# zyddnys/sd_animation_optical_flow

Measured on AMD Instinct MI355X. Metric: frame-pairs/sec (flow+warp+mask) at 512x768, higher is better.
Workload: dtype f32

## Files before the change

### include/ofx.h

```cpp
#ifndef OFX_H
#define OFX_H

#include <stddef.h>
#include <stdint.h>

#ifdef __cplusplus
extern "C" {
#endif

#define OFX_VERSION 100

#define OFX_EINVAL   (-1)
#define OFX_EALIGN   (-2)
#define OFX_ENOMEM   (-3)
#define OFX_EKEY     (-4)
#define OFX_ENODEV   (-5)

int ofx_version(void);
const char* ofx_error_string(int code);

int ofx_prof_enable(int on);
int ofx_prof_collect(char* json_out, size_t cap);

#define OFX_WARP_BILINEAR  0
// ... 109 lines not shown
#define OFX_EPI_FLOW    3

#define OFX_PREC_FP32   0
#define OFX_PREC_BF16X3 1
#define OFX_PREC_BF16X3_W 2
#define OFX_PREC_BF16X6_W 4
#define OFX_PREC_BF16X6 3
#define OFX_PREC_F16 5

typedef struct ofx_conv_desc {
    const float* in0; int ld0; int c0;
    const float* in1; int ld1; int c1;
    const float* w;
    const float* scale;
    const float* shift;
    float* out; int ldo;
    const float* res; int ldres;
    const float* nmean; const float* nrstd;
    const float* addend; int ldadd;
    float* aux_z; float* aux_rh; float* aux_h; int ldh;
    float* aux_coords; float* aux_flow4;
    long a_zs, w_zs, o_zs; int nz;
    int B, Hin, Win, Hout, Wout, Cout, KH, KW, stride, padH, padW;
    int act, epi;
    int tile;
    int precision;
    void* splitk_ws;
    size_t splitk_ws_bytes;
    const float* wino_w;
    const float* wino4_w;
} ofx_conv_desc;
#define OFX_CONV_TILE_WINOGRAD 1
#define OFX_CONV_TILE_WINOGRAD4 2

int ofx_conv2d(const ofx_conv_desc* d, void* stream);
typedef struct ofx_conv_plan {
    int path;
    int bm, bn, wm, wn, bk;
    int prec;
    int ks;
    int ksplit;
    int mode;
    int mtiles, ntiles, group_m;
    int stats_rows;
} ofx_conv_plan;
int ofx_conv2d_plan(const ofx_conv_desc* d, size_t stats_cap_floats, int want_pool, ofx_conv_plan* out);
long ofx_pack_conv_weight(const float* w_oihw, int Cout, int Cin, int KH, int KW, int cin_pad,
                          float* out);
int ofx_split_conv_weight(const float* packed, long n_floats, float* out);
long ofx_wino_conv_weight(const float* w_oihw, int Cout, int Cin, float* out);
long ofx_wino15_conv_weight(const float* w_oihw, int Cout, int Cin, int KH, int KW, float* out);
long ofx_wino44_conv_weight(const float* w_oihw, int Cout, int Cin, float* out);
int ofx_split_conv_weight3(const float* packed, long n_floats, float* out);

int ofx_inorm_stats(const float* x, int ld, float* mean, float* rstd, float* scratch,
                    int B, long HW, int C, float eps, void* stream);
int ofx_conv2d_stats(const ofx_conv_desc* d, float* part, size_t part_floats, int* rows_per_image, void* stream);
int ofx_inorm_finalize(const float* part, float* mean, float* rstd, int B, int rows, long HW, int C, float eps, void* stream);
int ofx_inorm_apply(const float* x, const float* mean, const float* rstd, const float* res,
                    const float* res_mean, const float* res_rstd, float* out, int B, long HW, int C,
                    int relu, void* stream);
int ofx_preprocess_u8(const uint8_t* img, float* out, long npix, int bgr, void* stream);

int ofx_corr_slice_floats(int h_l, int w_l);
int ofx_corr_volume(const float* f1, const float* f2, float* const* pyr, int B, int h, int w, int D,
                    int levels, void* stream);
// ... 75 lines not shown
```

### sd_animation_optical_flow_amd/csrc/conv.hip

```cpp
#include "ofx_internal.h"

#include <algorithm>
#include <cstdlib>
#include <cstring>
#include <type_traits>

namespace {

struct ConvK {
    const float* in0;
    const float* in1;
    const float* w;
    const float* scale;
    const float* shift;
    const float* addend;
    float* out;
    const float* res;
    const float* nmean;
    const float* nrstd;
    float* aux_z;
    float* aux_rh;
    float* aux_h;
    float* aux_coords;
    float* aux_flow4;
// ... 1090 lines not shown
        if (k.patch) return launch_tile_uk<BM, BN, WM, WN, BK, PREC, KS, SK, 2>(k, epi, norm, nz, s, ev);
    }
    if constexpr (tile_has_scalar(BN, PREC)) {
        if (k.uk) return launch_tile_uk<BM, BN, WM, WN, BK, PREC, KS, SK, 1>(k, epi, norm, nz, s, ev);
    }
    return launch_tile_uk<BM, BN, WM, WN, BK, PREC, KS, SK, 0>(k, epi, norm, nz, s, ev);
}

struct TileInst {
    int bm, bn, wm, wn, bk, prec, ks;
    bool sk;
    int (*launch)(const ConvK&, int epi, bool norm, int nz, hipStream_t, hipEvent_t);
};
#define OFX_TILE(BM, BN, WM, WN, BK, PREC, KS, SK) {BM, BN, WM, WN, BK, PREC, KS, SK, &launch_tile<BM, BN, WM, WN, BK, PREC, KS, SK>}
const TileInst kTiles[] = {
#ifndef OFX_CONV_LEAN
    OFX_TILE(128, 128, 64, 64, 16, 3, 1, false), OFX_TILE(128, 128, 64, 64, 16, 2, 1, false), OFX_TILE(128, 128, 64, 64, 16, 1, 1, false),
    OFX_TILE(128, 128, 64, 64, 16, 4, 1, false), OFX_TILE(128, 64, 64, 32, 16, 4, 1, false),  OFX_TILE(64, 64, 32, 32, 16, 4, 1, false),
    OFX_TILE(128, 64, 64, 32, 16, 3, 1, false),  OFX_TILE(64, 64, 32, 32, 16, 3, 1, false),   OFX_TILE(128, 128, 64, 64, 32, 1, 1, false),
    OFX_TILE(128, 64, 64, 32, 16, 2, 1, false),  OFX_TILE(128, 64, 64, 32, 16, 1, 1, false),  OFX_TILE(64, 64, 32, 32, 16, 2, 1, false),
    OFX_TILE(64, 64, 32, 32, 16, 1, 1, false),
    OFX_TILE(128, 128, 64, 64, 16, 5, 1, false), OFX_TILE(128, 64, 64, 32, 16, 5, 1, false),  OFX_TILE(64, 64, 32, 32, 16, 5, 1, false),
    OFX_TILE(128, 128, 64, 64, 32, 5, 1, false), OFX_TILE(128, 64, 64, 32, 32, 5, 1, false),  OFX_TILE(64, 64, 32, 32, 32, 5, 1, false),
#endif
    OFX_TILE(128, 128, 64, 64, 16, 0, 1, false), OFX_TILE(256, 64, 64, 64, 16, 0, 1, false),  OFX_TILE(128, 192, 64, 96, 16, 0, 1, false),
    OFX_TILE(128, 96, 32, 96, 16, 0, 1, false),  OFX_TILE(128, 64, 64, 32, 16, 0, 1, false),  OFX_TILE(128, 128, 64, 64, 32, 0, 1, false),
    OFX_TILE(128, 64, 64, 32, 32, 0, 1, false),  OFX_TILE(128, 32, 32, 32, 32, 0, 1, false),  OFX_TILE(64, 64, 32, 32, 16, 0, 1, false),
    OFX_TILE(64, 64, 32, 32, 32, 0, 1, true),    OFX_TILE(64, 64, 32, 32, 32, 0, 2, false),   OFX_TILE(64, 64, 32, 32, 32, 0, 1, false),
};
#undef OFX_TILE

struct ConvKnobs {
    bool no_wino = false, no_wino15 = false;
    bool no_wino44 = false;
    bool old_small = false;
    bool no_splitk = false;
    long sk_max_tiles = 2048;
    bool no_uk = false, no_patch = false;
    double patch_max_waste = 1.09;
    long vol_group_m = 0;
    long pair_max = 320;
    long f16_bk = 0;
};

const ConvKnobs& conv_knobs() {
    static const ConvKnobs knobs = [] {
        auto flag = [](const char* name) { return getenv(name) != nullptr; };
        auto number = [](const char* name, double lo, double hi, double dflt) {
            const char* e = getenv(name);
            char* end = nullptr;
            const double v = e ? strtod(e, &end) : 0.0;
            return e && end != e && !*end && v >= lo && v <= hi ? v : dflt;
        };
        ConvKnobs k;
        k.no_wino = flag("OFX_CONV_NO_WINOGRAD");
        k.no_wino15 = k.no_wino || flag("OFX_CONV_NO_WINOGRAD15");
        k.no_wino44 = k.no_wino || flag("OFX_CONV_NO_WINOGRAD4");
        k.old_small = flag("OFX_CONV_OLD_SMALL_TILES");
        k.no_splitk = flag("OFX_NO_SPLITK");
        k.no_uk = flag("OFX_CONV_NO_UK");
        k.no_patch = flag("OFX_CONV_NO_PATCH");
        auto count = [&](const char* name, long dflt) { const double v = number(name, 0, 0x7FFFFFFF, dflt); return v == (long)v ? (long)v : dflt; };
        k.sk_max_tiles = count("OFX_SK_MAX_TILES", k.sk_max_tiles);
        k.patch_max_waste = number("OFX_PATCH_MAX_WASTE", 1.0, 1e30, k.patch_max_waste);
        k.vol_group_m = count("OFX_VOL_GROUP_M", k.vol_group_m);
        k.pair_max = count("OFX_CONV_PAIR_MAX", k.pair_max);
        k.f16_bk = count("OFX_CONV_F16_BK", 0);
        if (k.f16_bk != 16 && k.f16_bk != 32) k.f16_bk = 0;
        return k;
    }();
    return knobs;
}

struct ConvPlan : ofx_conv_plan {
    int inst = -1;
    const char* name = nullptr;
    double flops = 0.0;
};

int conv_plan(const ofx_conv_desc* d, const ConvExtra& x, const ConvKnobs& kn, ConvPlan* p) {
    *p = ConvPlan{};
    p->ks = p->ksplit = p->group_m = 1;
    const int nz = d->nz > 1 ? d->nz : 1, cin = d->c0 + d->c1;
    const int K = d->KH * d->KW * cin, Kpad = ((K + kKAlign - 1) / kKAlign) * kKAlign;
    const long M = (long)d->B * d->Hout * d->Wout;
    const bool want_stats = x.stats_rows != nullptr, pool = x.pool.out != nullptr, fp32 = d->precision == OFX_PREC_FP32, f16 = d->precision == OFX_PREC_F16;
    p->name = nz > 1 ? "igemm_corr_volume"
              : d->epi == OFX_EPI_GRU_ZR ? "igemm_conv_gru_zr"
              : d->epi == OFX_EPI_GRU_Q  ? "igemm_conv_gru_q"
              : d->epi == OFX_EPI_FLOW   ? "igemm_conv_flow"
                                         : "igemm_conv";

    OfxWinoChoice wino;
    if (int st = ofx_conv_wino_choose(d, want_stats, x.stats_cap, pool, kn.no_wino, kn.no_wino15, kn.no_wino44, &wino)) return st;
    if (wino.path != kPathIgemm) {
        p->path = wino.path;
        p->stats_rows = wino.stats_rows;
        p->flops = wino.flops;
        return 0;
    }
    const bool one_d = (d->KH == 1 && d->KW == 5) || (d->KH == 5 && d->KW == 1);
    p->flops = 2.0 * (double)M * d->Cout * K * nz;

    int bm, bn;
    if (d->tile) {
        bm = (d->tile % 1000000) / 1000;
        bn = d->tile % 1000;
    } else {
        auto waste = [&](int t) { return (double)(((d->Cout + t - 1) / t) * t) / d->Cout; };
        if (d->Cout <= 32) bn = 32;
        else if (waste(128) <= 1.13 && !(waste(192) <= 1.0 && waste(128) > 1.05 && fp32 && !d->nmean && d->epi == OFX_EPI_PLAIN)) bn = 128;
        else if (waste(192) <= 1.05 && fp32 && !d->nmean && d->epi != OFX_EPI_FLOW) bn = 192;
        else if (waste(96) <= 1.05 && fp32 && d->epi == OFX_EPI_PLAIN) bn = 96;
        else if (waste(64) <= 1.13) bn = 64;
        else if (waste(32) < waste(64) - 0.1) bn = 32;
        else bn = 64;
        bm = 128;
        const long mt128 = (M + 127) / 128;
        auto blocks_of = [&](int t) { return mt128 * ((d->Cout + t - 1) / t) * nz; };
        constexpr long kFill = 768;
        const long blocks128 = blocks_of(bn);
        if (kn.old_small) {
            if (bn == 96 && blocks128 < 1024) bn = 32;
            if (bn >= 64 && blocks128 < 1024) bm = 64;
            if (bm == 64 && bn >= 128) bn = 64;
        } else if (bn >= 64 && blocks128 < kFill) {
            if (bn == 192 && d->epi == OFX_EPI_PLAIN && blocks_of(96) >= kFill) bn = 96;
            else if (bn >= 128 && blocks_of(64) >= kFill) bn = 64;
            else if (bn == 96) bn = 32;
// ... 183 lines not shown

int ofx_conv2d_ex(const ofx_conv_desc* d, const ConvExtra* extra, hipStream_t s) {
    const ConvExtra x = extra ? *extra : ConvExtra{};
    if (x.stats_rows) *x.stats_rows = 0;
    if (x.stop_taken) *x.stop_taken = false;
    long split_rows = 0;
    int st = conv_validate(d, x, &split_rows);
    if (st) return st;
    if (split_rows) {
        const long Mtot = (long)d->B * d->Hout * d->Wout;
        for (long r0 = 0; r0 < Mtot && !st; r0 += split_rows) {
            ofx_conv_desc part = *d;
            const long n = std::min(split_rows, Mtot - r0);
            part.B = 1; part.Hin = part.Hout = 1; part.Win = part.Wout = (int)n;
            part.in0 = d->in0 + r0 * d->ld0;
            if (d->in1) part.in1 = d->in1 + r0 * d->ld1;
            part.out = d->out + r0 * d->ldo;
            if (d->res) part.res = d->res + r0 * d->ldres;
            if (d->addend) part.addend = d->addend + r0 * d->ldadd;
            ConvExtra px;
            px.alpha = x.alpha;
            px.pool = x.pool;
            if (x.pool.out) px.pool.out = x.pool.out + r0 * x.pool.slice1;
            if (r0 + split_rows >= Mtot) { px.stop_event = x.stop_event; px.stop_taken = x.stop_taken; }
            st = ofx_conv2d_ex(&part, &px, s);
        }
        return st;
    }
    ConvPlan p;
    if ((st = conv_plan(d, x, conv_knobs(), &p))) return st;
    OfxProfScope prof(p.name, s);
    prof.flops(p.flops);
    if (p.path != kPathIgemm) {
        st = ofx_conv_wino_launch(d, p.path, x.alpha, p.stats_rows ? x.stats_part : nullptr, s, x.stop_event);
    } else {
        const bool pool = x.pool.out != nullptr;
        st = kTiles[p.inst].launch(conv_args(d, x, p), pool ? kEpiVolPool : d->epi, !pool && d->nmean != nullptr, d->nz > 1 ? d->nz : 1, s, x.stop_event);
    }
    if (st) return st;
    if (x.stats_rows) *x.stats_rows = p.stats_rows;
    if (x.stop_taken) *x.stop_taken = x.stop_event != nullptr;
    return 0;
}

extern "C" int ofx_conv2d(const ofx_conv_desc* d, void* stream) { return ofx_conv2d_ex(d, nullptr, (hipStream_t)stream); }

int ofx_conv2d_stats(const ofx_conv_desc* d, float* part, size_t part_floats, int* rows_per_image, void* stream) {
    OFX_REQUIRE(rows_per_image != nullptr, OFX_EINVAL);
    ConvExtra x;
    x.stats_part = part; x.stats_cap = part_floats; x.stats_rows = rows_per_image;
    return ofx_conv2d_ex(d, &x, (hipStream_t)stream);
}

extern "C" int ofx_conv2d_plan(const ofx_conv_desc* d, size_t stats_cap_floats, int want_pool, ofx_conv_plan* out) {
    OFX_REQUIRE(out != nullptr, OFX_EINVAL);
    int rows = 0;
    ConvExtra x;
    if (stats_cap_floats) { x.stats_cap = stats_cap_floats; x.stats_rows = &rows; }
    if (want_pool) { x.pool.out = reinterpret_cast<float*>(uintptr_t(16)); x.pool.wb0 = x.pool.wb1 = x.pool.slice1 = 1; }
    long split_rows = 0;
    int st = conv_validate(d, x, &split_rows);
    if (!st && split_rows) st = OFX_EINVAL;
    ConvPlan p;
    if (!st) st = conv_plan(d, x, conv_knobs(), &p);
    if (st) return st;
    *out = p;
    return 0;
// ... 65 lines not shown
```

### sd_animation_optical_flow_amd/csrc/conv_wino.hip

```cpp
#include "ofx_internal.h"

#include <cmath>
#include <cstdlib>
#include <cstring>

namespace {

constexpr int kWBK = 16;
constexpr int kLDV = kWBK + 4;
constexpr int kOOB = 0x7FFFFFF0;

template <int W_, int H_, int Y0, int X0> struct HaloGeom {
    static constexpr int W = W_, H = H_, y_org = Y0, x_org = X0;
    static constexpr int pix = W * H;
    static constexpr int items = pix * (kWBK / 4);
    static constexpr int slots = (items + 255) / 256;
};
template <bool VERT> struct Halo15 : HaloGeom<VERT ? 16 : 20, VERT ? 12 : 8, VERT ? -2 : 0, VERT ? 0 : -2> {
    static constexpr int ldh = VERT ? 16 : 20;
    static constexpr int floats = Halo15::pix * ldh;
    __device__ static int at(int pix) { return pix * ldh; }
};
struct Halo3x3 : HaloGeom<18, 10, -1, -1> {
    static constexpr int lpair = 36, lrow = 336;
// ... 483 lines not shown
            const float s12 = m1 + m2, d12 = m1 - m2, s34 = m3 + m4, d34 = m3 - m4, s56 = m5 + m6, d56 = m5 - m6;
            y[u][0] = m0 + s12 + s34 + s56;
            y[u][1] = d12 + 2.0f * d34 + 0.5f * d56;
            y[u][2] = s12 + 4.0f * s34 + 0.25f * s56;
            y[u][3] = d12 + 8.0f * d34 + 0.125f * d56 + m7;
        }
#pragma unroll
        for (int u = 0; u < 4; ++u)
#pragma unroll
            for (int i = 0; i < 4; ++i) {
                ad[u][i] = p.addend ? p.addend[pix[u][i] * p.ldadd + n] : 0.0f;
                x1[u][i] = EPI == OFX_EPI_GRU_ZR ? (r_half ? p.aux_h[pix[u][i] * p.ldh + n - hd] : 1.0f)
                           : EPI == OFX_EPI_GRU_Q ? p.aux_z[pix[u][i] * p.Cout + n] : 0.0f;
                x2[u][i] = EPI == OFX_EPI_GRU_Q ? p.aux_h[pix[u][i] * p.ldh + n] : 0.0f;
            }
#pragma unroll
        for (int u = 0; u < 4; ++u)
#pragma unroll
            for (int i = 0; i < 4; ++i) {
                const float v = y[u][i] * sc + sh + ad[u][i];
                if (EPI == OFX_EPI_PLAIN) {
                    p.out[pix[u][i] * p.ldo + n] = fmaxf(v, act_lo);
                } else if (EPI == OFX_EPI_GRU_ZR) {
                    const float g = ofx_sigmoid(v) * x1[u][i];
                    if (r_half) p.aux_rh[pix[u][i] * hd + n - hd] = g;
                    else p.aux_z[pix[u][i] * hd + n] = g;
                } else {
                    p.aux_h[pix[u][i] * p.ldh + n] = (1.0f - x1[u][i]) * x2[u][i] + x1[u][i] * ofx_tanh(v);
                }
            }
    }
}

struct Halo44 {
    static constexpr int W = 34, H = 18;
    static constexpr int lquad = 34, lrow = 308;
    static constexpr int floats = H * lrow;
    static constexpr int items = W * H * 2;
    static constexpr int threads = 768;
    static constexpr int slots = (items + threads - 1) / threads;
    __device__ __host__ static constexpr int at(int y, int x) { return y * lrow + (x >> 2) * lquad + (x & 3) * 8; }
    static constexpr int ltrow = 336;
    static constexpr int tfloats = 6 * 4 * ltrow;
    static constexpr int titems = 4 * W * 4;
};
constexpr int kLDX4 = 40;
constexpr int kXF4 = 12 * 4 * 16 * kLDX4;
constexpr int kStage44 = 2 * (Halo44::floats + Halo44::tfloats);
constexpr int kSmem44 = (kStage44 > kXF4 ? kStage44 : kXF4) * 4;
constexpr int kNorm44 = kSmem44 / 4 - kStage44;
constexpr int kNorm44MaxCin = kNorm44 / 2 / kWBK * kWBK;
constexpr int kSX4 = 2 * 24 * 32 * 2;
static_assert(kNorm44 >= 0 && kSX4 <= kXF4, "the fused options live in the plain kernel's LDS");

__global__ __launch_bounds__(768, 1) void wino44_conv_kernel(const WinoK p) {
    extern __shared__ __attribute__((aligned(16))) float smem44[];
    constexpr bool NORM = false, RES = false, STATS = false;
#include "conv_wino44_body.inl"
}

template <bool NORM, bool RES, bool STATS>
__global__ __launch_bounds__(768, 1) void wino44_fused_kernel(const WinoK p) {
    extern __shared__ __attribute__((aligned(16))) float smem44[];
#include "conv_wino44_body.inl"
}


using WinoKernel = void (*)(WinoK);

const WinoKernel kKernels22[8] = {wino_conv_kernel<false, false, false>, wino_conv_kernel<false, false, true>,
                                  wino_conv_kernel<false, true, false>,  nullptr,
                                  wino_conv_kernel<true, false, false>,  wino_conv_kernel<true, false, true>,
                                  wino_conv_kernel<true, true, false>,   nullptr};
const WinoKernel kKernels15[8] = {wino15_conv_kernel<true, OFX_EPI_PLAIN>,  wino15_conv_kernel<true, OFX_EPI_GRU_ZR>,
                                  wino15_conv_kernel<true, OFX_EPI_GRU_Q>,  wino15_conv_kernel<false, OFX_EPI_PLAIN>,
                                  wino15_conv_kernel<false, OFX_EPI_GRU_ZR>, wino15_conv_kernel<false, OFX_EPI_GRU_Q>,
                                  nullptr,                                  nullptr};
const WinoKernel kKernels44[8] = {wino44_conv_kernel,                       wino44_fused_kernel<false, false, true>,
                                  wino44_fused_kernel<false, true, false>,  nullptr,
                                  wino44_fused_kernel<true, false, false>,  wino44_fused_kernel<true, false, true>,
                                  wino44_fused_kernel<true, true, false>,   nullptr};

struct WinoAlg {
    bool one_d;
    int ph, pw;
    int points, outputs;
    int cblk;
    int threads, dyn_lds;
    const float* ofx_conv_desc::*u;
    int tile;
    long min_grid;
    bool per_block;
    bool gates;
    bool norm_pair;
    int norm_max_cin;
    int path, path_fused;
    const WinoKernel* kernels;
};

const WinoAlg kAlgs[] = {
    {false, 16, 32, 36, 16, 64, 768, kSmem44, &ofx_conv_desc::wino4_w, OFX_CONV_TILE_WINOGRAD4, 768, true,
     false, true, kNorm44MaxCin, kPathWino44, kPathWino44Fused, kKernels44},
    {false, 8, 16, 16, 4, 64, 256, 0, &ofx_conv_desc::wino_w, OFX_CONV_TILE_WINOGRAD, 1024, true,
     false, false, 0x7FFFFFFF, kPathWino3x3, kPathWino3x3, kKernels22},
    {true, 8, 16, 8, 4, 128, 256, 0, &ofx_conv_desc::wino_w, OFX_CONV_TILE_WINOGRAD, 256, false,
     true, false, 0, kPathWino15, kPathWino15, kKernels15},
};
constexpr int kNumAlgs = sizeof kAlgs / sizeof kAlgs[0];

bool is_1d(int KH, int KW) { return (KH == 1 && KW == 5) || (KH == 5 && KW == 1); }

bool wino_fits(const WinoAlg& a, const ofx_conv_desc* d) {
    const int cin = d->c0 + d->c1;
    const float* const u = d->*a.u;
    const bool plain = d->epi == OFX_EPI_PLAIN && d->out != nullptr && d->ldo >= d->Cout && (d->act == OFX_ACT_NONE || d->act == OFX_ACT_RELU);
    const bool shape = a.one_d ? is_1d(d->KH, d->KW) : d->KH == 3 && d->KW == 3;
    bool epi;
    if (a.gates) {
        epi = !d->nmean && !d->res && (plain || (d->epi == OFX_EPI_GRU_ZR && (d->Cout / 2) % a.cblk == 0) || d->epi == OFX_EPI_GRU_Q);
    } else {
        epi = plain && !d->addend && (!d->res || d->ldres >= d->Cout) && (!a.norm_pair || (d->nmean != nullptr) == (d->nrstd != nullptr)) &&
              (!d->nmean || (d->nrstd && !d->in1 && d->c0 <= a.norm_max_cin && ofx_aligned16(d->nmean) && ofx_aligned16(d->nrstd)));
    }
    return shape && epi && d->padH == d->KH / 2 && d->padW == d->KW / 2 && d->precision == OFX_PREC_FP32 && d->nz <= 1 && d->stride == 1 &&
           d->Hout == d->Hin && d->Wout == d->Win && d->Hin % a.ph == 0 && d->Win % a.pw == 0 && cin % kWBK == 0 && d->c0 % kWBK == 0 &&
           u != nullptr && ofx_aligned16(u);
}

int wino_stats_rows(const WinoAlg& a, const ofx_conv_desc* d) {
    return !a.gates && d->act == OFX_ACT_NONE && !d->res ? (d->Hin / a.ph) * (d->Win / a.pw) : 0;
}

int wino_args(const WinoAlg& a, const ofx_conv_desc* d, float alpha, float* stats, WinoK* out) {
    WinoK k{};
    k.in0 = d->in0; k.in1 = d->in1; k.u = d->*a.u; k.scale = d->scale; k.shift = d->shift; k.addend = d->addend; k.out = d->out;
    k.res = d->res; k.nmean = d->nmean; k.nrstd = d->nrstd; k.stats = stats;
    k.aux_z = d->aux_z; k.aux_rh = d->aux_rh; k.aux_h = d->aux_h;
    k.ld0 = d->ld0; k.c0 = d->c0; k.ld1 = d->ld1; k.cin = d->c0 + d->c1; k.ldo = d->ldo; k.ldadd = d->ldadd; k.ldh = d->ldh;
    k.ldres = d->ldres;
    k.H = d->Hin; k.W = d->Win; k.Cout = d->Cout; k.act = d->act;
    k.nblk = (d->Cout + a.cblk - 1) / a.cblk;
    k.nb32 = a.cblk / 32 * k.nblk;
    k.tpr = d->Win / a.pw;
    k.tpi = (d->Hin / a.ph) * k.tpr;
    const long mtiles = (long)d->B * k.tpi;
    const long npix = (long)d->B * d->Hin * d->Win;
    const long ext0 = ((npix - 1) * d->ld0 + d->c0) * 4, ext1 = d->in1 ? ((npix - 1) * d->ld1 + d->c1) * 4 : 0;
    const long extu = (long)a.points * k.nb32 * 32 * k.cin * 4;
    OFX_REQUIRE(ext0 < (1L << 31) - 64 && ext1 < (1L << 31) - 64 && extu < (1L << 31) - 64, OFX_EINVAL);
    OFX_REQUIRE(mtiles * k.nblk < (1L << 31) && (a.one_d || npix * d->ldo < (1L << 31)), OFX_EINVAL);
    k.mtiles = (int)mtiles;
    k.bytes0 = (int)ext0; k.bytes1 = (int)ext1; k.bytesu = (int)extu;
    k.alpha = alpha;
    *out = k;
    return 0;
}

int wino_launch_kernel(const WinoAlg& a, int v, const WinoK& k, hipStream_t s, hipEvent_t stop_event) {
    const WinoKernel kernel = v >= 0 && v < 8 ? a.kernels[v] : nullptr;
    OFX_REQUIRE(kernel != nullptr, OFX_EINVAL);
    if (a.dyn_lds > 65536) {
        static bool allowed[64][kNumAlgs][8] = {};
        int dev = 0;
        if (hipGetDevice(&dev) != hipSuccess || dev < 0 || dev >= 64) return OFX_EINVAL;
        bool& ok = allowed[dev][&a - kAlgs][v];
        if (!ok) {
            const hipError_t e = hipFuncSetAttribute(reinterpret_cast<const void*>(kernel), hipFuncAttributeMaxDynamicSharedMemorySize, a.dyn_lds);
            if (e != hipSuccess) return (int)e;
            ok = true;
        }
    }
    const dim3 grid((unsigned)(k.mtiles * k.nblk), 1, 1), block(a.threads, 1, 1);
    if (stop_event) hipExtLaunchKernelGGL(kernel, grid, block, a.dyn_lds, s, nullptr, stop_event, 0, k);
    else hipLaunchKernelGGL(kernel, grid, block, a.dyn_lds, s, k);
    return ofx_launch_status();
}

}

int ofx_conv_wino_choose(const ofx_conv_desc* d, bool want_stats, size_t stats_cap, bool pool, bool no_wino, bool no_wino15, bool no_wino44,
                         OfxWinoChoice* c) {
    *c = OfxWinoChoice{};
    const bool off[kNumAlgs] = {no_wino44, no_wino, no_wino15};
    const bool one_d = is_1d(d->KH, d->KW);
    for (int i = 0; i < kNumAlgs; ++i) {
        const WinoAlg& a = kAlgs[i];
        const bool force = d->tile == a.tile;
        if (a.one_d != one_d || !(force || (d->tile == 0 && !off[i] && d->*a.u))) continue;
        const int srows = want_stats ? wino_stats_rows(a, d) : 0;
        const bool stats_ok = !want_stats || (srows > 0 && (size_t)d->B * srows * d->Cout * 2 <= stats_cap);
        if (!(stats_ok && !pool && wino_fits(a, d))) continue;
        const long patches = (long)d->B * (d->Hin / a.ph) * (d->Win / a.pw);
        if (!force && patches * (a.per_block ? (d->Cout + a.cblk - 1) / a.cblk : 1) < a.min_grid) continue;
        c->path = want_stats || d->res || d->nmean || d->nrstd ? a.path_fused : a.path;
        c->stats_rows = srows;
        c->flops = 2.0 * a.points * ((double)d->B * d->Hout * d->Wout / a.outputs) * (double)(d->c0 + d->c1) * d->Cout;
        return 0;
    }
    return d->tile == OFX_CONV_TILE_WINOGRAD || d->tile == OFX_CONV_TILE_WINOGRAD4 ? OFX_EINVAL : 0;
}

int ofx_conv_wino_launch(const ofx_conv_desc* d, int path, float alpha, float* stats, hipStream_t s, hipEvent_t stop_event) {
    const WinoAlg* a = nullptr;
    for (const WinoAlg& row : kAlgs)
        if (path == row.path || path == row.path_fused) a = &row;
    OFX_REQUIRE(a && (!stats || wino_stats_rows(*a, d) > 0), OFX_EINVAL);
    WinoK k;
    if (int st = wino_args(*a, d, alpha, stats, &k)) return st;
    const int v = a->gates ? (d->epi >= OFX_EPI_PLAIN && d->epi <= OFX_EPI_GRU_Q ? (d->KH == 5 ? 0 : 3) + d->epi : -1)
                           : (k.nmean ? 4 : 0) | (k.res ? 2 : 0) | (k.stats ? 1 : 0);
    return wino_launch_kernel(*a, v, k, s, stop_event);
}

namespace {

template <class XF>
long wino_weight(const float* w, int Cout, int Cin, int taps, int points, int cblk, float* out, XF xf) {
    OFX_REQUIRE(Cout > 0 && Cin > 0 && Cin % kWBK == 0, OFX_EINVAL);
    const int nb32 = cblk / 32 * ((Cout + cblk - 1) / cblk);
    const long n = (long)points * nb32 * 32 * Cin;
    if (!out) return n;
    OFX_REQUIRE(w != nullptr, OFX_EINVAL);
    std::memset(out, 0, (size_t)n * sizeof(float));
    double u[16];
    for (int o = 0; o < Cout; ++o)
        for (int c = 0; c < Cin; ++c) {
            xf(w + ((size_t)o * Cin + c) * taps, u);
            for (int q = 0; q < points; ++q) {
                const long at = ((((long)q * nb32 + o / 32) * (Cin / 8) + c / 8) * 2 + (c % 8) / 4) * 128 + 4 * (o % 32) + c % 4;
                out[at] = (float)u[q];
            }
        }
    return n;
}

}

extern "C" long ofx_wino_conv_weight(const float* w, int Cout, int Cin, float* out) {
// ... 56 lines not shown
```

### sd_animation_optical_flow_amd/csrc/ofx_internal.h

```cpp
#pragma once
#include <hip/hip_runtime.h>
#include <stdint.h>
#include <stddef.h>
#include "../../include/ofx.h"

#define OFX_HIP_CHECK(expr)                         \
    do {                                            \
        hipError_t _e = (expr);                     \
        if (_e != hipSuccess) return (int)_e;       \
    } while (0)

#define OFX_REQUIRE(cond, code) \
    do {                        \
        if (!(cond)) return (code); \
    } while (0)

static inline bool ofx_aligned16(const void* p) { return (((uintptr_t)p) & 15u) == 0; }
static inline int ofx_cdiv(long a, long b) { return (int)((a + b - 1) / b); }

void ofx_prof_set_tag(const char* tag);
struct OfxProfScope {
    int slot;
    hipStream_t stream;
    OfxProfScope(const char* name, hipStream_t s);
    ~OfxProfScope();
    void flops(double f);
};

#ifdef __HIPCC__
#include <hip/hip_ext.h>
#define OFX_LAUNCH(kern, grid, block, s, ev, ...)                                                  \
    do {                                                                                           \
        if (ev) {                                                                                  \
            hipExtLaunchKernelGGL(kern, grid, block, 0, s, nullptr, ev, 0, __VA_ARGS__);           \
        } else {                                                                                   \
            hipLaunchKernelGGL(kern, grid, block, 0, s, __VA_ARGS__);                              \
        }                                                                                          \
    } while (0)
#endif

static inline int ofx_launch_status() {
    hipError_t e = hipGetLastError();
    return (int)e;
}

struct ConvExtra {
    float alpha = 1.0f;
    struct Pool { float* out = nullptr; long zs = 0; int wb0 = 0, wb1 = 0, slice1 = 0; } pool;
    float* stats_part = nullptr;
    size_t stats_cap = 0;
    int* stats_rows = nullptr;
    hipEvent_t stop_event = nullptr;
    bool* stop_taken = nullptr;
};
int ofx_conv2d_ex(const ofx_conv_desc* d, const ConvExtra* extra, hipStream_t s);
enum { kPathIgemm = 0, kPathWino3x3 = 1, kPathWino15 = 2, kPathWino44 = 3, kPathWino44Fused = 4 };
struct OfxWinoChoice {
    int path = kPathIgemm, stats_rows = 0;
    double flops = 0.0;
};
int ofx_conv_wino_choose(const ofx_conv_desc* d, bool want_stats, size_t stats_cap, bool pool, bool no_wino, bool no_wino15, bool no_wino44,
                         OfxWinoChoice* c);
int ofx_conv_wino_launch(const ofx_conv_desc* d, int path, float alpha, float* stats, hipStream_t s, hipEvent_t stop_event);

int ofx_inorm_finalize_part(const float* part, float* mean, float* rstd, int B, int rows, long HW, int C, float eps, hipStream_t s,
                            const float* gamma = nullptr, const float* beta = nullptr);
int ofx_inorm_stats_affine(const float* x, int ld, float* mean, float* rstd, float* scratch, int B, long HW, int C, float eps,
                           const float* gamma, const float* beta, hipStream_t stream);

int ofx_groupnorm_launch(const float* x0, int ld0, int C0, const float* x1, int ld1, int C1, const float* e, int lde, const float* gamma,
                         const float* beta, float* out, void* scratch, int B, long HW, int groups, float eps, int silu,
                         const char* const scope[3], hipStream_t s);

bool ofx_attention_flash_ok(int D);
int ofx_attention_flash_launch(const float* q, const float* k, const float* v, const float* bias, long bias_bstride, float* out, int BH, int Nq,
                               int Nk, int D, float scale, int precision, hipStream_t s);
int ofx_attention_flash_bnhd_launch(const float* q, int ldq, const float* k, int ldk, const float* v, int ldv, const float* bias,
                                    long bias_bstride, float* out, int ldo, int B, int H, int Nq, int Nk, int D, float scale, int precision,
                                    hipStream_t s);

int ofx_local_corr_launch(const float* f1, const float* f2, const float* coords, float* out, long sb, long sn,
                          long sc, long sp, int B, int H1, int W1, int H2, int W2, int C, int N, int r, float scale,
                          float cscale, hipStream_t s);
int ofx_local_corr_tiled_launch(const float* f1, const float* const* f2l, const int* idx1, const int* idx2, const float* coords, float* out,
                                int ld, int B, int h, int w, int C, int r, int levels, float scale, hipStream_t s);
int ofx_corr_slice_floats_l(int hl, int wl);
int ofx_corr_lookup_pad(const float* const* pyr, const float* coords, float* out, int ldo, int pad, int B, int h, int w, int levels,
                        int radius, void* stream);
int ofx_corr_block_rows(const float* src, float* dst, int n, int h, int w, int D, hipStream_t s);
int ofx_corr_pool_launch(const float* l0, float* l1, float* l2, float* l3, int B, int h, int w, int levels, hipStream_t s,
                         bool from_l1 = false);
bool ofx_corr_volpool_ok(int h, int w);
bool ofx_corr_volsplit_ok(int h, int w, int D);
bool ofx_corr_volsplit_pays(int nz, int h, int w, int planes);
size_t ofx_corr_planes_bytes(int h, int w, int planes);
int ofx_corr_split_planes(const float* src, void* dst, int n, int h, int w, int planes, int quad, float alpha, hipStream_t s);
// ... 48 lines not shown
```

### sd_animation_optical_flow_amd/ops.py

```python
from __future__ import annotations

import ctypes as C
import json
import math
from typing import Dict, List, Optional, Sequence, Tuple

import torch

from . import _lib
from ._lib import ConvDesc, check

WARP_MODES = {"bilinear": 0, "bicubic": 1, "cv2_cubic": 2}
ACTS = {None: 0, "none": 0, "relu": 1, "sigmoid": 2, "tanh": 3}
EPI_PLAIN, EPI_GRU_ZR, EPI_GRU_Q, EPI_FLOW = 0, 1, 2, 3
TILE_WINOGRAD = 1
TILE_WINOGRAD4 = 2


def _stream() -> C.c_void_p:
    return C.c_void_p(torch.cuda.current_stream().cuda_stream)


def _chk(t: torch.Tensor, name: str, dtype=None) -> torch.Tensor:
    if not isinstance(t, torch.Tensor):
        raise RuntimeError(f"{name} must be a torch.Tensor")
    if not t.is_cuda:
        raise RuntimeError(f"{name} must be a CUDA tensor")
    if not t.is_contiguous():
        raise RuntimeError(f"{name} must be contiguous")
    if dtype is not None and t.dtype != dtype:
        raise RuntimeError(f"{name} must be {dtype}, got {t.dtype}")
    return t


def _ptr(t: Optional[torch.Tensor]) -> C.c_void_p:
    return C.c_void_p(0 if t is None else t.data_ptr())


def prof_enable(on) -> None:
    check(_lib.lib().ofx_prof_enable(int(on)), "ofx_prof_enable")


def prof_collect() -> dict:
    buf = C.create_string_buffer(1 << 18)
    check(_lib.lib().ofx_prof_collect(buf, len(buf)), "ofx_prof_collect")
    return json.loads(buf.value.decode())


def warp(frame: torch.Tensor, flow: torch.Tensor, mode: str = "bilinear", sign: float = 1.0) -> torch.Tensor:
# ... 1002 lines not shown
```

Baseline: 363.8.

## Add wide 256-channel Winograd 1x5/5x1 kernel with dual K-slice subgroups

Adds a new Winograd kernel for the 1x5/5x1 GRU convolutions. Each 512-thread block covers 256 output channels, split into two 4-wave subgroups that each take alternating input-channel slices and transform their own halo into separate LDS regions. The weight fragments are preloaded in registers and prefetched across iterations. Each wave reads A fragments from both subgroups' LDS, so a single output tile sums the whole K range without a cross-wave reduction. The new kernel is tried before the existing 128-channel wino15 path when Cout divides 256 and cin divides 2*kWBK. Choice and launch now pass the algorithm row index instead of the path id. This reuses each input transform across more output channels per block, at the cost of heavy register use and single-block occupancy.

```diff
diff --git a/include/ofx.h b/include/ofx.h
--- a/include/ofx.h
+++ b/include/ofx.h
@@ -165,6 +165,7 @@
 } ofx_conv_desc;
 #define OFX_CONV_TILE_WINOGRAD 1
 #define OFX_CONV_TILE_WINOGRAD4 2
+#define OFX_CONV_TILE_WINOGRAD15_WIDE 3
 
 int ofx_conv2d(const ofx_conv_desc* d, void* stream);
 typedef struct ofx_conv_plan {
diff --git a/sd_animation_optical_flow_amd/csrc/conv.hip b/sd_animation_optical_flow_amd/csrc/conv.hip
--- a/sd_animation_optical_flow_amd/csrc/conv.hip
+++ b/sd_animation_optical_flow_amd/csrc/conv.hip
@@ -1146,6 +1146,7 @@
 
 struct ConvKnobs {
     bool no_wino = false, no_wino15 = false;
+    bool no_wino15w = false;
     bool no_wino44 = false;
     bool old_small = false;
     bool no_splitk = false;
@@ -1169,6 +1170,7 @@
         ConvKnobs k;
         k.no_wino = flag("OFX_CONV_NO_WINOGRAD");
         k.no_wino15 = k.no_wino || flag("OFX_CONV_NO_WINOGRAD15");
+        k.no_wino15w = k.no_wino15 || flag("OFX_CONV_NO_WINOGRAD15_WIDE");
         k.no_wino44 = k.no_wino || flag("OFX_CONV_NO_WINOGRAD4");
         k.old_small = flag("OFX_CONV_OLD_SMALL_TILES");
         k.no_splitk = flag("OFX_NO_SPLITK");
@@ -1188,6 +1190,7 @@
 
 struct ConvPlan : ofx_conv_plan {
     int inst = -1;
+    int wino_row = -1;
     const char* name = nullptr;
     double flops = 0.0;
 };
@@ -1206,9 +1209,10 @@
                                          : "igemm_conv";
 
     OfxWinoChoice wino;
-    if (int st = ofx_conv_wino_choose(d, want_stats, x.stats_cap, pool, kn.no_wino, kn.no_wino15, kn.no_wino44, &wino)) return st;
+    if (int st = ofx_conv_wino_choose(d, want_stats, x.stats_cap, pool, kn.no_wino, kn.no_wino15, kn.no_wino15w, kn.no_wino44, &wino)) return st;
     if (wino.path != kPathIgemm) {
         p->path = wino.path;
+        p->wino_row = wino.row;
         p->stats_rows = wino.stats_rows;
         p->flops = wino.flops;
         return 0;
@@ -1458,7 +1462,7 @@
     OfxProfScope prof(p.name, s);
     prof.flops(p.flops);
     if (p.path != kPathIgemm) {
-        st = ofx_conv_wino_launch(d, p.path, x.alpha, p.stats_rows ? x.stats_part : nullptr, s, x.stop_event);
+        st = ofx_conv_wino_launch(d, p.wino_row, x.alpha, p.stats_rows ? x.stats_part : nullptr, s, x.stop_event);
     } else {
         const bool pool = x.pool.out != nullptr;
         st = kTiles[p.inst].launch(conv_args(d, x, p), pool ? kEpiVolPool : d->epi, !pool && d->nmean != nullptr, d->nz > 1 ? d->nz : 1, s, x.stop_event);
diff --git a/sd_animation_optical_flow_amd/csrc/conv_wino.hip b/sd_animation_optical_flow_amd/csrc/conv_wino.hip
--- a/sd_animation_optical_flow_amd/csrc/conv_wino.hip
+++ b/sd_animation_optical_flow_amd/csrc/conv_wino.hip
@@ -539,6 +539,167 @@
     }
 }
 
+template <bool VERT> constexpr int kSub15 = Halo15<VERT>::floats + 8 * 32 * kLDV;
+constexpr int kSmem15W = 2 * (kSub15<false> > kSub15<true> ? kSub15<false> : kSub15<true>) * 4;
+
+template <bool VERT, int EPI>
+__global__ __launch_bounds__(512, 1) void wino15_wide_kernel(const WinoK p) {
+    using T = Wino15<VERT>;
+    using HALO = typename T::HALO;
+    extern __shared__ __attribute__((aligned(16))) float smem15w[];
+    const int tid = threadIdx.x, lane = tid & 63;
+    const int wave = __builtin_amdgcn_readfirstlane(tid >> 6);
+    const int sub = wave >> 2, tid2 = tid & 255;
+    float* const Hs = smem15w + sub * kSub15<VERT>;
+    float* const Vs = Hs + HALO::floats;
+    const Patch pt = wino_patch(p);
+
+    const float* in1s = p.in1 ? p.in1 : p.in0;
+    const int bytes1s = p.in1 ? p.bytes1 : p.bytes0;
+    int hpix[HALO::slots];
+    unsigned hok = 0;
+#pragma unroll
+    for (int k = 0; k < HALO::slots; ++k) {
+        const int i = tid2 + 256 * k;
+        const int pix = i >> 2;
+        const int hy = pix / HALO::W, hx = pix - hy * HALO::W;
+        const int gy = pt.y0 + HALO::y_org + hy, gx = pt.x0 + HALO::x_org + hx;
+        const bool ok = i < HALO::items && (unsigned)gy < (unsigned)p.H && (unsigned)gx < (unsigned)p.W;
+        hpix[k] = ok ? (pt.pb * p.H + gy) * p.W + gx : 0;
+        hok |= (ok ? 1u : 0u) << k;
+    }
+    const int hq = (tid2 & 3) * 16;
+    float4 pa[HALO::slots];
+    auto a_issue = [&](int trip) __attribute__((always_inline)) {
+        const int c = (2 * trip + sub) * kWBK;
+        const bool s0 = c < p.c0;
+        const __amdgpu_buffer_rsrc_t rs = __builtin_amdgcn_make_buffer_rsrc((void*)(s0 ? p.in0 : in1s), (short)0, s0 ? p.bytes0 : bytes1s, 0x00020000);
+        const int so = (s0 ? c : c - p.c0) * 4;
+        const int ldb = (s0 ? p.ld0 : p.ld1) * 4;
+#pragma unroll
+        for (int k = 0; k < HALO::slots; ++k) {
+            const int vo = ((hok >> k) & 1u) ? hpix[k] * ldb + hq : kOOB;
+            v4i t = __builtin_amdgcn_raw_buffer_load_b128(rs, vo, so, 0);
+            pa[k] = *reinterpret_cast<float4*>(&t);
+        }
+    };
+
+    const __amdgpu_buffer_rsrc_t rsu = __builtin_amdgcn_make_buffer_rsrc((void*)p.u, (short)0, p.bytesu, 0x00020000);
+    const int c8n = p.cin >> 3;
+    const int wlane = lane * 16;
+    const int blk0 = 8 * pt.nb + wave;
+    float4 wr[16];
+    auto w_issue = [&](int i, int c8) __attribute__((always_inline)) {
+        const int so = (((i >> 1) * p.nb32 + blk0) * c8n + c8 + (i & 1)) * 1024;
+        v4i t = __builtin_amdgcn_raw_buffer_load_b128(rsu, wlane, so, 0);
+        wr[i] = *reinterpret_cast<float4*>(&t);
+    };
+
+    f32x16 acc[8];
+#pragma unroll
+    for (int q = 0; q < 8; ++q)
+#pragma unroll
+        for (int e = 0; e < 16; ++e) acc[q][e] = 0.f;
+
+    const T xf(Hs, Vs, tid2, wave);
+    const float* const afrag = smem15w + HALO::floats + (lane & 31) * kLDV + 4 * (lane >> 5);
+    auto a_read = [&](int j) __attribute__((always_inline)) {
+        return *reinterpret_cast<const float4*>(afrag + (j >> 4) * kSub15<VERT> + ((j & 15) >> 1) * 32 * kLDV + 8 * (j & 1));
+    };
+
+    const int TB = p.cin / (2 * kWBK);
+    a_issue(0);
+#pragma unroll
+    for (int i = 0; i < 16; ++i) {
+        w_issue(i, 0);
+        __builtin_amdgcn_sched_barrier(0);
+    }
+    for (int tb = 0; tb < TB; ++tb) {
+        const int nx = tb + 1 < TB ? tb + 1 : tb;
+#pragma unroll
+        for (int k = 0; k < HALO::slots; ++k) {
+            const int i = tid2 + 256 * k;
+            if (HALO::slots * 256 > HALO::items && k == HALO::slots - 1 && i >= HALO::items) break;
+            float4 v = pa[k];
+            *reinterpret_cast<float4*>(&Hs[HALO::at(i >> 2) + (i & 3) * 4]) = v;
+        }
+        __syncthreads();
+        xf();
+        __syncthreads();
+        a_issue(nx);
+        __builtin_amdgcn_sched_barrier(0);
+        float4 a[32];
+        a[0] = a_read(0);
+        a[1] = a_read(1);
+        __builtin_amdgcn_sched_group_barrier(0x100, 2, 0);
+#pragma unroll
+        for (int j = 0; j < 32; ++j) {
+            const int i = j & 15, q = i >> 1;
+            if (j + 2 < 32) a[j + 2] = a_read(j + 2);
+            const float4 b = wr[i];
+            acc[q] = __builtin_amdgcn_mfma_f32_32x32x2f32(a[j].x, b.x, acc[q], 0, 0, 0);
+            acc[q] = __builtin_amdgcn_mfma_f32_32x32x2f32(a[j].y, b.y, acc[q], 0, 0, 0);
+            acc[q] = __builtin_amdgcn_mfma_f32_32x32x2f32(a[j].z, b.z, acc[q], 0, 0, 0);
+            acc[q] = __builtin_amdgcn_mfma_f32_32x32x2f32(a[j].w, b.w, acc[q], 0, 0, 0);
+            w_issue(i, j < 16 ? 4 * tb + 2 : 4 * nx);
+            if (j + 2 < 32) __builtin_amdgcn_sched_group_barrier(0x100, 1, 0);
+            __builtin_amdgcn_sched_group_barrier(0x008, 4, 0);
+            __builtin_amdgcn_sched_group_barrier(0x020, 1, 0);
+        }
+    }
+
+    const int n = pt.nb * 256 + wave * 32 + (lane & 31);
+    if (n >= p.Cout) return;
+    const float sc = (p.scale ? p.scale[n] : 1.0f) * p.alpha;
+    const float sh = p.shift ? p.shift[n] : 0.0f;
+    const float act_lo = p.act == OFX_ACT_RELU ? 0.0f : -3.402823466e38f;
+    const int hd = p.Cout >> 1;
+    const bool r_half = EPI == OFX_EPI_GRU_ZR && pt.nb * 256 + wave * 32 >= hd;
+#pragma unroll
+    for (int eb = 0; eb < 16; eb += 4) {
+        long pix[4][4];
+        float y[4][4], ad[4][4], x1[4][4], x2[4][4];
+#pragma unroll
+        for (int u = 0; u < 4; ++u) {
+            const int e = eb + u;
+            const int tile = (e & 3) + 8 * (e >> 2) + 4 * (lane >> 5);
+#pragma unroll
+            for (int i = 0; i < 4; ++i) pix[u][i] = ((long)pt.pb * p.H + pt.y0 + T::oy(tile, i)) * p.W + pt.x0 + T::ox(tile, i);
+            const float m0 = acc[0][e], m1 = acc[1][e], m2 = acc[2][e], m3 = acc[3][e];
+            const float m4 = acc[4][e], m5 = acc[5][e], m6 = acc[6][e], m7 = acc[7][e];
+            const float s12 = m1 + m2, d12 = m1 - m2, s34 = m3 + m4, d34 = m3 - m4, s56 = m5 + m6, d56 = m5 - m6;
+            y[u][0] = m0 + s12 + s34 + s56;
+            y[u][1] = d12 + 2.0f * d34 + 0.5f * d56;
+            y[u][2] = s12 + 4.0f * s34 + 0.25f * s56;
+            y[u][3] = d12 + 8.0f * d34 + 0.125f * d56 + m7;
+        }
+#pragma unroll
+        for (int u = 0; u < 4; ++u)
+#pragma unroll
+            for (int i = 0; i < 4; ++i) {
+                ad[u][i] = p.addend ? p.addend[pix[u][i] * p.ldadd + n] : 0.0f;
+                x1[u][i] = EPI == OFX_EPI_GRU_ZR ? (r_half ? p.aux_h[pix[u][i] * p.ldh + n - hd] : 1.0f)
+                           : EPI == OFX_EPI_GRU_Q ? p.aux_z[pix[u][i] * p.Cout + n] : 0.0f;
+                x2[u][i] = EPI == OFX_EPI_GRU_Q ? p.aux_h[pix[u][i] * p.ldh + n] : 0.0f;
+            }
+#pragma unroll
+        for (int u = 0; u < 4; ++u)
+#pragma unroll
+            for (int i = 0; i < 4; ++i) {
+                const float v = y[u][i] * sc + sh + ad[u][i];
+                if (EPI == OFX_EPI_PLAIN) {
+                    p.out[pix[u][i] * p.ldo + n] = fmaxf(v, act_lo);
+                } else if (EPI == OFX_EPI_GRU_ZR) {
+                    const float g = ofx_sigmoid(v) * x1[u][i];
+                    if (r_half) p.aux_rh[pix[u][i] * hd + n - hd] = g;
+                    else p.aux_z[pix[u][i] * hd + n] = g;
+                } else {
+                    p.aux_h[pix[u][i] * p.ldh + n] = (1.0f - x1[u][i]) * x2[u][i] + x1[u][i] * ofx_tanh(v);
+                }
+            }
+    }
+}
+
 struct Halo44 {
     static constexpr int W = 34, H = 18;
     static constexpr int lquad = 34, lrow = 308;
@@ -583,6 +744,10 @@
                                   wino15_conv_kernel<true, OFX_EPI_GRU_Q>,  wino15_conv_kernel<false, OFX_EPI_PLAIN>,
                                   wino15_conv_kernel<false, OFX_EPI_GRU_ZR>, wino15_conv_kernel<false, OFX_EPI_GRU_Q>,
                                   nullptr,                                  nullptr};
+const WinoKernel kKernels15W[8] = {wino15_wide_kernel<true, OFX_EPI_PLAIN>,  wino15_wide_kernel<true, OFX_EPI_GRU_ZR>,
+                                   wino15_wide_kernel<true, OFX_EPI_GRU_Q>,  wino15_wide_kernel<false, OFX_EPI_PLAIN>,
+                                   wino15_wide_kernel<false, OFX_EPI_GRU_ZR>, wino15_wide_kernel<false, OFX_EPI_GRU_Q>,
+                                   nullptr,                                  nullptr};
 const WinoKernel kKernels44[8] = {wino44_conv_kernel,                       wino44_fused_kernel<false, false, true>,
                                   wino44_fused_kernel<false, true, false>,  nullptr,
                                   wino44_fused_kernel<true, false, false>,  wino44_fused_kernel<true, false, true>,
@@ -593,6 +758,9 @@
     int ph, pw;
     int points, outputs;
     int cblk;
+    bool whole_cblk;
+    int trip;
+    int zr_split;
     int threads, dyn_lds;
     const float* ofx_conv_desc::*u;
     int tile;
@@ -606,15 +774,16 @@
 };
 
 const WinoAlg kAlgs[] = {
-    {false, 16, 32, 36, 16, 64, 768, kSmem44, &ofx_conv_desc::wino4_w, OFX_CONV_TILE_WINOGRAD4, 768, true,
+    {false, 16, 32, 36, 16, 64, false, kWBK, 0, 768, kSmem44, &ofx_conv_desc::wino4_w, OFX_CONV_TILE_WINOGRAD4, 768, true,
      false, true, kNorm44MaxCin, kPathWino44, kPathWino44Fused, kKernels44},
-    {false, 8, 16, 16, 4, 64, 256, 0, &ofx_conv_desc::wino_w, OFX_CONV_TILE_WINOGRAD, 1024, true,
+    {false, 8, 16, 16, 4, 64, false, kWBK, 0, 256, 0, &ofx_conv_desc::wino_w, OFX_CONV_TILE_WINOGRAD, 1024, true,
      false, false, 0x7FFFFFFF, kPathWino3x3, kPathWino3x3, kKernels22},
-    {true, 8, 16, 8, 4, 128, 256, 0, &ofx_conv_desc::wino_w, OFX_CONV_TILE_WINOGRAD, 256, false,
+    {true, 8, 16, 8, 4, 256, true, 2 * kWBK, 32, 512, kSmem15W, &ofx_conv_desc::wino_w, OFX_CONV_TILE_WINOGRAD15_WIDE, 768, true,
+     true, false, 0, kPathWino15, kPathWino15, kKernels15W},
+    {true, 8, 16, 8, 4, 128, false, kWBK, 128, 256, 0, &ofx_conv_desc::wino_w, OFX_CONV_TILE_WINOGRAD, 256, false,
      true, false, 0, kPathWino15, kPathWino15, kKernels15},
 };
 constexpr int kNumAlgs = sizeof kAlgs / sizeof kAlgs[0];
-
 bool is_1d(int KH, int KW) { return (KH == 1 && KW == 5) || (KH == 5 && KW == 1); }
 
 bool wino_fits(const WinoAlg& a, const ofx_conv_desc* d) {
@@ -624,14 +793,14 @@
     const bool shape = a.one_d ? is_1d(d->KH, d->KW) : d->KH == 3 && d->KW == 3;
     bool epi;
     if (a.gates) {
-        epi = !d->nmean && !d->res && (plain || (d->epi == OFX_EPI_GRU_ZR && (d->Cout / 2) % a.cblk == 0) || d->epi == OFX_EPI_GRU_Q);
+        epi = !d->nmean && !d->res && (plain || (d->epi == OFX_EPI_GRU_ZR && (d->Cout / 2) % a.zr_split == 0) || d->epi == OFX_EPI_GRU_Q);
     } else {
         epi = plain && !d->addend && (!d->res || d->ldres >= d->Cout) && (!a.norm_pair || (d->nmean != nullptr) == (d->nrstd != nullptr)) &&
               (!d->nmean || (d->nrstd && !d->in1 && d->c0 <= a.norm_max_cin && ofx_aligned16(d->nmean) && ofx_aligned16(d->nrstd)));
     }
     return shape && epi && d->padH == d->KH / 2 && d->padW == d->KW / 2 && d->precision == OFX_PREC_FP32 && d->nz <= 1 && d->stride == 1 &&
-           d->Hout == d->Hin && d->Wout == d->Win && d->Hin % a.ph == 0 && d->Win % a.pw == 0 && cin % kWBK == 0 && d->c0 % kWBK == 0 &&
-           u != nullptr && ofx_aligned16(u);
+           d->Hout == d->Hin && d->Wout == d->Win && d->Hin % a.ph == 0 && d->Win % a.pw == 0 && cin % a.trip == 0 && d->c0 % a.trip == 0 &&
+           (!a.whole_cblk || d->Cout % a.cblk == 0) && u != nullptr && ofx_aligned16(u);
 }
 
 int wino_stats_rows(const WinoAlg& a, const ofx_conv_desc* d) {
@@ -685,10 +854,10 @@
 
 }
 
-int ofx_conv_wino_choose(const ofx_conv_desc* d, bool want_stats, size_t stats_cap, bool pool, bool no_wino, bool no_wino15, bool no_wino44,
-                         OfxWinoChoice* c) {
+int ofx_conv_wino_choose(const ofx_conv_desc* d, bool want_stats, size_t stats_cap, bool pool, bool no_wino, bool no_wino15, bool no_wino15w,
+                         bool no_wino44, OfxWinoChoice* c) {
     *c = OfxWinoChoice{};
-    const bool off[kNumAlgs] = {no_wino44, no_wino, no_wino15};
+    const bool off[kNumAlgs] = {no_wino44, no_wino, no_wino15w, no_wino15};
     const bool one_d = is_1d(d->KH, d->KW);
     for (int i = 0; i < kNumAlgs; ++i) {
         const WinoAlg& a = kAlgs[i];
@@ -700,17 +869,16 @@
         const long patches = (long)d->B * (d->Hin / a.ph) * (d->Win / a.pw);
         if (!force && patches * (a.per_block ? (d->Cout + a.cblk - 1) / a.cblk : 1) < a.min_grid) continue;
         c->path = want_stats || d->res || d->nmean || d->nrstd ? a.path_fused : a.path;
+        c->row = i;
         c->stats_rows = srows;
         c->flops = 2.0 * a.points * ((double)d->B * d->Hout * d->Wout / a.outputs) * (double)(d->c0 + d->c1) * d->Cout;
         return 0;
     }
-    return d->tile == OFX_CONV_TILE_WINOGRAD || d->tile == OFX_CONV_TILE_WINOGRAD4 ? OFX_EINVAL : 0;
-}
-
-int ofx_conv_wino_launch(const ofx_conv_desc* d, int path, float alpha, float* stats, hipStream_t s, hipEvent_t stop_event) {
-    const WinoAlg* a = nullptr;
-    for (const WinoAlg& row : kAlgs)
-        if (path == row.path || path == row.path_fused) a = &row;
+    return d->tile == OFX_CONV_TILE_WINOGRAD || d->tile == OFX_CONV_TILE_WINOGRAD4 || d->tile == OFX_CONV_TILE_WINOGRAD15_WIDE ? OFX_EINVAL : 0;
+}
+
+int ofx_conv_wino_launch(const ofx_conv_desc* d, int row, float alpha, float* stats, hipStream_t s, hipEvent_t stop_event) {
+    const WinoAlg* a = row >= 0 && row < kNumAlgs ? &kAlgs[row] : nullptr;
     OFX_REQUIRE(a && (!stats || wino_stats_rows(*a, d) > 0), OFX_EINVAL);
     WinoK k;
     if (int st = wino_args(*a, d, alpha, stats, &k)) return st;
diff --git a/sd_animation_optical_flow_amd/csrc/ofx_internal.h b/sd_animation_optical_flow_amd/csrc/ofx_internal.h
--- a/sd_animation_optical_flow_amd/csrc/ofx_internal.h
+++ b/sd_animation_optical_flow_amd/csrc/ofx_internal.h
@@ -56,12 +56,12 @@
 int ofx_conv2d_ex(const ofx_conv_desc* d, const ConvExtra* extra, hipStream_t s);
 enum { kPathIgemm = 0, kPathWino3x3 = 1, kPathWino15 = 2, kPathWino44 = 3, kPathWino44Fused = 4 };
 struct OfxWinoChoice {
-    int path = kPathIgemm, stats_rows = 0;
+    int path = kPathIgemm, row = -1, stats_rows = 0;
     double flops = 0.0;
 };
-int ofx_conv_wino_choose(const ofx_conv_desc* d, bool want_stats, size_t stats_cap, bool pool, bool no_wino, bool no_wino15, bool no_wino44,
-                         OfxWinoChoice* c);
-int ofx_conv_wino_launch(const ofx_conv_desc* d, int path, float alpha, float* stats, hipStream_t s, hipEvent_t stop_event);
+int ofx_conv_wino_choose(const ofx_conv_desc* d, bool want_stats, size_t stats_cap, bool pool, bool no_wino, bool no_wino15, bool no_wino15w,
+                         bool no_wino44, OfxWinoChoice* c);
+int ofx_conv_wino_launch(const ofx_conv_desc* d, int row, float alpha, float* stats, hipStream_t s, hipEvent_t stop_event);
 
 int ofx_inorm_finalize_part(const float* part, float* mean, float* rstd, int B, int rows, long HW, int C, float eps, hipStream_t s,
                             const float* gamma = nullptr, const float* beta = nullptr);
diff --git a/sd_animation_optical_flow_amd/ops.py b/sd_animation_optical_flow_amd/ops.py
--- a/sd_animation_optical_flow_amd/ops.py
+++ b/sd_animation_optical_flow_amd/ops.py
@@ -15,6 +15,7 @@
 EPI_PLAIN, EPI_GRU_ZR, EPI_GRU_Q, EPI_FLOW = 0, 1, 2, 3
 TILE_WINOGRAD = 1
 TILE_WINOGRAD4 = 2
+TILE_WINOGRAD15_WIDE = 3
 
 
 def _stream() -> C.c_void_p:
```

Measured after the change: 366.7, median of 6. No clear change (+0.8%).
